# risingwavelabs/risingwave

Measured on NVIDIA H100. Metric: Nexmark q7/q8-shaped streaming HashJoin input rows/s, higher is better.
Workload: dtype int64

## Files before the change

risingwave_b200/csrc/join.cu:

```cuda
#include <algorithm>
#include <cstdio>
#include <cstdlib>
#include <memory>
#include <mutex>
#include <thread>

#include <cub/device/device_radix_sort.cuh>
#include <cub/device/device_scan.cuh>

#include "common.cuh"

namespace rw {

#define J_EMPTY 0x8000000000000000ull
#define J_NIL 0x7fffffffu
#define J_DEAD 0x80000000u
#define J_MAX_OUT (2 * RW_MAX_COLS)
#define J_HDR 16
#define W_EMPTY 0x7fffffffull
#define W_COUNT_ONE (1ull << 33)
#define W_IL_LIVE (1ull << 31)
#define W_IL_DEAD (2ull << 31)
#define W_IL_MASK (3ull << 31)
__device__ __host__ __forceinline__ uint32_t W_head(uint64_t W) { return (uint32_t)(W & 0x7fffffffull); }
// ... 24 lines not shown
  int out_type[J_MAX_OUT];
  int out_width[J_MAX_OUT];
  int n_map[2];
  int map_in[2][J_MAX_OUT];
  int map_out[2][J_MAX_OUT];
  int need_degree[2];
  int append_only_optimize;
  int cond_cmp, cond_lhs, cond_rhs;
  int single_key, KW, SW;
  int strict;
};

struct JoinSideDev {
  uint8_t* recs;
  uint8_t* buckets;
  uint64_t cap;
  int stride;
  int bstride;
};

struct JoinStatus {
  unsigned long long out_rows;
  unsigned long long n_store;
  unsigned long long n_del;
  unsigned long long null_mask;
  unsigned long long n_keys[2];
  unsigned int err;
  unsigned int pad;
  unsigned long long n_in;
  unsigned long long log_next[2];
  unsigned long long n_dead[2];
  unsigned long long n_defer;
};

struct JoinOutDev {
  uint8_t* ops;
  uint8_t* vis;
  void* col[J_MAX_OUT];
  uint8_t* valid[J_MAX_OUT];
  int64_t capacity;
  const uint8_t* heap[2];
};

__device__ __host__ __forceinline__ bool jt_is_outer_side(int T, int S) { return T == RW_JOIN_FULL_OUTER || (T == RW_JOIN_LEFT_OUTER && S == 0) || (T == RW_JOIN_RIGHT_OUTER && S == 1); }
__device__ __host__ __forceinline__ bool jt_outer_side_null(int T, int S) { return T == RW_JOIN_FULL_OUTER || (T == RW_JOIN_LEFT_OUTER && S == 1) || (T == RW_JOIN_RIGHT_OUTER && S == 0); }
__device__ __host__ __forceinline__ bool jt_forward_exactly_once(int T, int S) { return ((T == RW_JOIN_LEFT_SEMI || T == RW_JOIN_LEFT_ANTI) && S == 0) || ((T == RW_JOIN_RIGHT_SEMI || T == RW_JOIN_RIGHT_ANTI) && S == 1); }
__device__ __host__ __forceinline__ bool jt_only_forward_matched_side(int T, int S) { return ((T == RW_JOIN_LEFT_SEMI || T == RW_JOIN_LEFT_ANTI) && S == 1) || ((T == RW_JOIN_RIGHT_SEMI || T == RW_JOIN_RIGHT_ANTI) && S == 0); }
__device__ __host__ __forceinline__ bool jt_is_semi(int T) { return T == RW_JOIN_LEFT_SEMI || T == RW_JOIN_RIGHT_SEMI; }
__device__ __host__ __forceinline__ bool jt_is_anti(int T) { return T == RW_JOIN_LEFT_ANTI || T == RW_JOIN_RIGHT_ANTI; }
__device__ __host__ __forceinline__ bool jt_forward_if_not_matched(int T, int S) { return (jt_is_anti(T) && jt_forward_exactly_once(T, S)) || jt_is_outer_side(T, S); }

struct RecHdr {
  uint32_t link, nullmask, seq, degree;
};
__device__ __forceinline__ uint8_t* rec_ptr(const JoinSideDev& s, uint32_t row) { return s.recs + (uint64_t)row * s.stride; }
__device__ __forceinline__ RecHdr* rec_hdr(const JoinSideDev& s, uint32_t row) { return (RecHdr*)rec_ptr(s, row); }

__device__ __forceinline__ uint64_t rec_key_word(const uint8_t* rec, int off, int width, int type) {
  ColRef cr;
  cr.data = rec + off;
  cr.valid_bits = nullptr;
  cr.valid_bytes = nullptr;
  cr.type = type;
  cr.width = width;
  return load_key_word(cr, 0);
}
// ... 1203 lines not shown
      if (!sg.p) {
        cudaError_t e = sg.reserve((size_t)U_SEG_RECS * 48);
        if (e != cudaSuccess) { cudaGetLastError(); return fail(RW_ERR_OOM, std::string("join log segment: ") + cudaGetErrorString(e)); }
        stalls++;
      }
      void* ptr = sg.p;
      RW_CUDA(cudaMemcpyAsync(table.as<uint8_t>() + segs.size() * sizeof(void*), &ptr, sizeof(void*), cudaMemcpyHostToDevice, st));
      segs.push_back(std::move(sg));
    }
    return RW_OK;
  }
};

struct JoinSideHost {
  int n_cols = 0;
  std::vector<int> types;
  SegLog log;
  GrowBuf recs;
  DevBuf slots;
  DevBuf pools;
  int stride = 0, bstride = 0;
  uint64_t row_cap = 0;
  uint64_t n_rows = 0;
  uint64_t slot_cap = 0;
  uint64_t keys_upper = 0;
};

struct JoinPending {
  int S = 0, set = 0, grid = 0;
  DevChunk ch;
  cudaStream_t st = nullptr;
  int64_t out_base = 0;
  bool plain = true, counted = false, sync_done = false;
  bool alias_u = false;
  uint32_t pool_chunk = 0;
  uint64_t seq_base = 0, ids_before = 0, keys_before = 0;
  unsigned long long tag = 0;
  int64_t rows = 0;
  unsigned long long nullm = 0;
};

struct rwgpu_join {
  JoinPlanDev plan;
  DevBuf plan_dev, status;
  PinnedBuf status_host;
  JoinSideHost side[2];
  cudaStream_t stream = nullptr, s_h2d = nullptr, s_d2h = nullptr;
  cudaEvent_t ev_h2d[8] = {nullptr}, ev_main[8] = {nullptr};
  std::vector<int> out_types;
  int chunk_size = 1024;
  bool fast_inner = false;
  bool w8_ok[2] = {false, false};
  W8Plan w8[2];
  bool uni = false;
  int uni_is = 1;
  DevBuf uni_buckets, uni_counters;
  uint64_t uni_cap = 0, uni_keys = 0, uni_keys_exact = 0;
  uint64_t uni_dead[2] = {0, 0};
  uint64_t compactions = 0;
  DevBuf uni_wk_entry, uni_wk_mask;
  int64_t uni_wk_cap = 0;
  JoinPending pending[2];
  int n_pending = 0;
  cudaEvent_t pend_ev[2] = {nullptr, nullptr};
  cudaStream_t last_st = nullptr;
  cudaEvent_t order_ev = nullptr;
  bool wm_pending[2] = {false, false};
  int wm_key_pos[2] = {0, 0};
  int64_t wm_value[2] = {0, 0};
  uint64_t wm_cleanings = 0;
  uint64_t launches = 0;
  uint64_t seq = 0;
  unsigned long long status_tag = 0;
  unsigned long long call_null_mask = 0;
  bool out_rows_cumulative = false;
  KernelProf prof;
  DevBuf sk, sk_alt, packed, offs, mslot, gtable, cub_tmp;
  int64_t scratch_rows = 0;
  uint64_t gcap = 0;
  size_t cub_bytes = 0;
  struct OutSet {
    DevBuf out_ops, out_vis, out_col[J_MAX_OUT], out_valid[J_MAX_OUT], out_bits[J_MAX_OUT], out_visbits;
    int64_t out_cap = 0;
    unsigned long long valid_dirty = 0;
  } oset[2];
  int cur = 0;
  OutSet& os() { return oset[cur]; }
  struct HostPending {
    bool active = false;
    rwgpu_out* out = nullptr;
    std::vector<rw_column> in_cols;
    std::vector<int> alias_src;
    int64_t n = 0, host_cap = 0;
  } hpend[2];
// ... 154 lines not shown

static JoinOutDev out_dev(rwgpu_join* h) {
  JoinOutDev o;
  memset(&o, 0, sizeof(o));
  o.ops = h->os().out_ops.as<uint8_t>();
  o.vis = h->os().out_vis.as<uint8_t>();
  for (size_t k = 0; k < h->out_types.size(); k++) { o.col[k] = h->os().out_col[k].p; o.valid[k] = h->os().out_valid[k].as<uint8_t>(); }
  o.capacity = h->os().out_cap;
  o.heap[0] = h->var_heap[0].as<uint8_t>();
  o.heap[1] = h->var_heap[1].as<uint8_t>();
  return o;
}

__global__ void join_status_to_host_kernel(JoinStatus* src, JoinStatus* dst_host, unsigned long long tag, int reset) {
  join_status_publish(src, dst_host, tag, reset);
}
static int join_read_status(rwgpu_join* h, cudaStream_t st, JoinStatus* out, int reset = 1, unsigned long long tag = 0) {
  JoinStatus* host = h->status_host.as<JoinStatus>();
  if (tag) {
    RW_CUDA(cudaStreamSynchronize(st));
    if (*(volatile unsigned long long*)(host + 1) == tag) {
      memcpy(out, host, sizeof(JoinStatus));
      return RW_OK;
    }
  }
  join_status_to_host_kernel<<<1, 1, 0, st>>>(h->status.as<JoinStatus>(), host, 0ull, reset);
  RW_CUDA(cudaGetLastError());
  h->launches++;
  RW_CUDA(cudaStreamSynchronize(st));
  memcpy(out, host, sizeof(JoinStatus));
  return RW_OK;
}

static int join_check_err(rwgpu_join* h, const JoinStatus& s, cudaStream_t st) {
  if (!s.err) return RW_OK;
  unsigned int e = s.err;
  cudaMemsetAsync(&h->status.as<JoinStatus>()->err, 0, sizeof(unsigned int), st);
  if (e & JERR_DOUBLE_DELETE) return fail(RW_ERR_INCONSISTENT, "removing a join state entry but it is not in the cache");
  if (e & JERR_APPEND_ONLY_MULTI) return fail(RW_ERR_INCONSISTENT, "append-only optimisation: more than one matched row");
  if (e & JERR_STORE_CAPACITY) return fail(RW_ERR_CUDA, "internal: join record store capacity");
  if (e & JERR_BAD_COUNT) return fail(RW_ERR_INVALID, "device row count out of range");
  return fail(RW_ERR_CUDA, "internal: join output capacity");
}

static UniDev uni_dev(rwgpu_join* h) {
  UniDev t;
  t.buckets = h->uni_buckets.as<uint8_t>();
  t.cap = h->uni_cap;
  unsigned long long* ctr = h->uni_counters.as<unsigned long long>();
  for (int s = 0; s < 2; s++) {
    t.log[s] = h->side[s].log.table.as<uint8_t*>();
    t.log_cap[s] = h->side[s].log.cap();
    t.pools[s] = h->side[s].pools.as<uint2>();
    t.log_next[s] = ctr + s;
    t.n_dead[s] = ctr + 2 + s;
  }
  t.is = h->uni_is;
  return t;
}

static int uni_alloc_buckets(rwgpu_join* h, DevBuf& buf, uint64_t cap) {
  RW_CUDA(buf.reserve((cap + 2) * 64));
  uni_init_kernel<<<jgrid((int64_t)cap + 2, 256), 256, 0, h->stream>>>(buf.as<uint8_t>(), 0, cap + 2);
  RW_CUDA(cudaGetLastError());
  h->launches++;
  return RW_OK;
}

static int uni_grow_table(rwgpu_join* h, uint64_t need_keys) {
  if (need_keys * U_LOAD_INV <= h->uni_cap) return RW_OK;
  if (h->uni_keys_exact * U_LOAD_INV <= h->uni_cap && need_keys * 10 <= h->uni_cap * 9) return RW_OK;
  uint64_t ncap = h->uni_cap;
  while (ncap < need_keys * 2 * U_LOAD_INV) ncap <<= 1;
  RW_CUDA(cudaDeviceSynchronize());
  DevBuf nb;
  int rc = uni_alloc_buckets(h, nb, ncap);
  if (rc != RW_OK) return rc;
  uni_rehash_kernel<<<jgrid((int64_t)h->uni_cap + 2, 256), 256, 0, h->stream>>>(h->uni_buckets.as<uint8_t>(), h->uni_cap, nb.as<uint8_t>(), ncap);
  RW_CUDA(cudaGetLastError());
  h->launches++;
  RW_CUDA(cudaStreamSynchronize(h->stream));
  h->uni_buckets = std::move(nb);
  h->uni_cap = ncap;
  return RW_OK;
}

static int uni_compact(rwgpu_join* h, int s) {
  JoinSideHost& sd = h->side[s];
  RW_CUDA(cudaDeviceSynchronize());
  SegLog fresh;
  const uint64_t live_upper = sd.n_rows > h->uni_dead[s] ? sd.n_rows - h->uni_dead[s] : 0;
  int rc = fresh.ensure(std::max<uint64_t>(live_upper, 1), h->stream);
  if (rc != RW_OK) { set_error(""); return RW_OK; }
  unsigned long long* ctr = h->uni_counters.as<unsigned long long>();
  RW_CUDA(cudaMemsetAsync(ctr + 4, 0, 8, h->stream));
  uni_compact_kernel<<<jgrid((int64_t)h->uni_cap + 2, 256), 256, 0, h->stream>>>(uni_dev(h), s, fresh.table.as<uint8_t*>(), ctr + 4);
  RW_CUDA(cudaGetLastError());
  h->launches++;
  unsigned long long live = 0;
  RW_CUDA(cudaMemcpyAsync(&live, ctr + 4, 8, cudaMemcpyDeviceToHost, h->stream));
  RW_CUDA(cudaStreamSynchronize(h->stream));
  std::swap(sd.log.segs, fresh.segs);
  {
    DevBuf t2 = std::move(sd.log.table);
    sd.log.table = std::move(fresh.table);
    fresh.table = std::move(t2);
// ... 5 lines not shown
  RW_CUDA(cudaMemcpyAsync(ctr + s, &live, 8, cudaMemcpyHostToDevice, h->stream));
  RW_CUDA(cudaMemcpyAsync(ctr + 2 + s, &zero, 8, cudaMemcpyHostToDevice, h->stream));
  RW_CUDA(cudaMemsetAsync(sd.pools.p, 0, sd.pools.bytes, h->stream));
  RW_CUDA(cudaStreamSynchronize(h->stream));
  h->compactions++;
  return RW_OK;
}

static int join_order(rwgpu_join* h, cudaStream_t st) {
  if (h->last_st && h->last_st != st) {
    if (!h->order_ev) RW_CUDA(cudaEventCreateWithFlags(&h->order_ev, cudaEventDisableTiming));
    RW_CUDA(cudaEventRecord(h->order_ev, h->last_st));
    RW_CUDA(cudaStreamWaitEvent(st, h->order_ev, 0));
  }
  h->last_st = st;
  return RW_OK;
}

static int uni_tail_grid(int64_t n) {
  static int max_blocks = 0;
  if (!max_blocks) {
    int dev = 0, sms = 0, per_sm = 0;
    cudaGetDevice(&dev);
    cudaDeviceGetAttribute(&sms, cudaDevAttrMultiProcessorCount, dev);
    int a = 0, b = 0;
    cudaOccupancyMaxActiveBlocksPerMultiprocessor(&a, uni_tail_kernel<false>, 256, 0);
    cudaOccupancyMaxActiveBlocksPerMultiprocessor(&b, uni_tail_kernel<true>, 256, 0);
    per_sm = std::max(1, std::min(std::min(a, b), 3));
    max_blocks = std::max(1, sms * per_sm);
  }
  return (int)std::max<int64_t>(1, std::min<int64_t>((n + 255) / 256, max_blocks));
}

static int uni_launch_main(rwgpu_join* h, const JoinPending& pd, bool probe_only, unsigned long long tag) {
  UniDev t = uni_dev(h);
  const JoinPlanDev* pdev = h->plan_dev.as<JoinPlanDev>();
  JoinStatus* ds = h->status.as<JoinStatus>();
  int S = pd.S;
  const bool is_row = S == h->uni_is;
  JoinOutDev od = out_dev(h);
  UniWork wk;
  wk.entry = h->uni_wk_entry.as<UniDefer>();
  wk.mask = h->uni_wk_mask.as<uint8_t>();
  W8Plan w = h->w8[S];
  h->prof.begin(pd.st);
  if (pd.plain) {
    PlainChunk pc;
    pc.ops = pd.ch.ops;
    for (int c = 0; c < 4; c++) pc.c[c] = c < w.n_u ? (const unsigned long long*)pd.ch.cols[c].data : nullptr;
    pc.key = (const unsigned long long*)pd.ch.cols[w.key_col].data;
    pc.n = pd.ch.n;
    pc.n_dev = pd.ch.n_dev;
    UniOwn own;
    own.log = t.log[S];
    own.log_cap = t.log_cap[S];
    own.pools = t.pools[S];
    own.log_next = t.log_next[S];
    PlainOut po;
    po.ops = od.ops;
    po.vis = od.vis;
    const int mkey = pd.alias_u ? h->w8[1 - S].key_col : -1;
    for (int c = 0; c < 4; c++) {
      po.ucol[c] = (!pd.alias_u && c < w.n_u && w.u_out[c] >= 0) ? (unsigned long long*)od.col[w.u_out[c]] : nullptr;
      po.mcol[c] = (c != mkey && c < w.n_m && w.m_out[c] >= 0) ? (unsigned long long*)od.col[w.m_out[c]] : nullptr;
    }
    po.capacity = od.capacity;
    auto hot = probe_only ? (is_row ? uni_hot_kernel<true, true> : uni_hot_kernel<true, false>)
                          : (is_row ? uni_hot_kernel<false, true> : uni_hot_kernel<false, false>);
    hot<<<pd.grid, JF_BLOCK, 0, pd.st>>>(pc, t.buckets, t.cap, own, po, wk, ds, pd.seq_base, pd.out_base, pd.pool_chunk);
  } else {
    if (probe_only) uni_slow_kernel<true><<<jgrid(pd.ch.n, 256), 256, 0, pd.st>>>(pdev, w, S, pd.ch, t, od, ds, pd.seq_base, pd.out_base);
    else uni_slow_kernel<false><<<jgrid(pd.ch.n, 256), 256, 0, pd.st>>>(pdev, w, S, pd.ch, t, od, ds, pd.seq_base, pd.out_base);
  }
  h->prof.end(pd.st);
  RW_CUDA(cudaGetLastError());
  DevChunk chv = pd.ch;
  uint64_t seq_base = pd.seq_base;
  int64_t out_base = pd.out_base;
  JoinStatus* slot = (JoinStatus*)(h->status_host.as<uint8_t>() + 512 * pd.set);
  int reset = 3;
  unsigned int* done = (unsigned int*)(h->uni_counters.as<unsigned long long>() + 6);
  const int tg = uni_tail_grid(pd.ch.n);
  if (probe_only) uni_tail_kernel<true><<<tg, 256, 0, pd.st>>>(pdev, w, S, chv, t, od, wk, ds, seq_base, out_base, slot, tag, reset, done);
  else uni_tail_kernel<false><<<tg, 256, 0, pd.st>>>(pdev, w, S, chv, t, od, wk, ds, seq_base, out_base, slot, tag, reset, done);
  RW_CUDA(cudaGetLastError());
  h->launches += 2;
  return RW_OK;
}

static int join_plain_chunk(DevChunk* ch, bool device_count, cudaStream_t st, bool* plain) {
  *plain = ch->vis_bits == nullptr;
  for (int c = 0; c < ch->n_cols && *plain; c++)
    *plain = !ch->cols[c].valid_bits && !ch->cols[c].valid_bytes && (((uintptr_t)ch->cols[c].data & 7) == 0);
  if (!ch->n_dev || (device_count && *plain)) return RW_OK;
  int64_t nh = 0;
  RW_CUDA(cudaMemcpyAsync(&nh, ch->n_dev, sizeof(nh), cudaMemcpyDeviceToHost, st));
  RW_CUDA(cudaStreamSynchronize(st));
  if (nh < 0 || nh > ch->n) return fail(RW_ERR_INVALID, "device row count out of range");
  ch->n = nh;
  ch->n_dev = nullptr;
  return RW_OK;
}

static int uni_enqueue(rwgpu_join* h, int S, const DevChunk& ch_in, cudaStream_t st, int64_t out_base, bool alias_ok, JoinPending* pd) {
  DevChunk ch = ch_in;
  bool plain_cols;
  int rc = join_plain_chunk(&ch, true, st, &plain_cols);
  if (rc != RW_OK) return rc;
  const bool counted = ch.n_dev != nullptr;
  const int64_t n = ch.n;
  JoinSideHost& own = h->side[S];
  const int grid = (int)std::max<int64_t>(1, std::min<int64_t>((n + 63) / 64, U_MAX_GRID));
  uint32_t pool_chunk = 32;
  while (pool_chunk < 256 && (int64_t)pool_chunk * grid * 8 < 4 * n) pool_chunk <<= 1;
  const uint64_t id_slack = (uint64_t)grid * 8 * pool_chunk;
  rc = join_grow_store(h, S, own.n_rows + (uint64_t)n + id_slack);
  if (rc != RW_OK) return rc;
  rc = uni_grow_table(h, h->uni_keys + (uint64_t)n);
  if (rc != RW_OK) return rc;
  rc = join_ensure_out(h, out_base + n + std::max<int64_t>(n / 2, 4096), st, out_base);
  if (rc != RW_OK) return rc;
  if (plain_cols && n > h->uni_wk_cap) {
    RW_CUDA(cudaDeviceSynchronize());
    const int64_t cap = n + n / 4 + 64;
    RW_CUDA(h->uni_wk_entry.reserve((size_t)cap * sizeof(UniDefer)));
    RW_CUDA(h->uni_wk_mask.reserve((size_t)(cap + 7) / 8 + 16));
    h->uni_wk_cap = cap;
  }
  rc = join_order(h, st);
  if (rc != RW_OK) return rc;
  pd->S = S;
  pd->ch = ch;
  pd->st = st;
  pd->out_base = out_base;
  pd->set = h->cur;
  pd->plain = plain_cols;
  pd->counted = counted;
  pd->alias_u = alias_ok && plain_cols && !counted && out_base == 0 && h->var_in[S].empty();
  pd->grid = grid;
  pd->pool_chunk = pool_chunk;
  pd->seq_base = h->seq;
  pd->tag = ++h->status_tag;
  pd->ids_before = own.n_rows;
  pd->keys_before = h->uni_keys;
  h->seq += (uint64_t)n;
  own.n_rows += (uint64_t)n + id_slack;
  h->uni_keys += (uint64_t)n;
  rc = uni_launch_main(h, *pd, false, pd->tag);
  if (rc != RW_OK) return rc;
  if (!h->pend_ev[pd->set]) RW_CUDA(cudaEventCreateWithFlags(&h->pend_ev[pd->set], cudaEventDisableTiming));
  RW_CUDA(cudaEventRecord(h->pend_ev[pd->set], st));
  return RW_OK;
}

static int uni_finish(rwgpu_join* h, const JoinPending& pd, int64_t* out_rows, unsigned long long* null_mask, bool* aliased = nullptr) {
  cudaStream_t st = pd.st;
  JoinStatus* ds = h->status.as<JoinStatus>();
  JoinStatus* slot = (JoinStatus*)(h->status_host.as<uint8_t>() + 512 * pd.set);
  JoinStatus hs;
  RW_CUDA(cudaEventSynchronize(h->pend_ev[pd.set]));
  int rc;
  if (*(volatile unsigned long long*)(slot + 1) != pd.tag) return fail(RW_ERR_CUDA, "join status block was not published");
  memcpy(&hs, slot, sizeof(JoinStatus));
  unsigned int err = hs.err;
  const unsigned long long first_null = hs.null_mask;
  const bool first_match = hs.pad != 0;
  const unsigned long long first_del = hs.n_del;
  const bool redone = (hs.err & JERR_OUT_CAPACITY) != 0;
  if (redone) {
    const int64_t extras = (int64_t)hs.out_rows, n = pd.ch.n;
    RW_CUDA(cudaMemsetAsync(&ds->err, 0, 4, st));
    rc = join_ensure_out(h, pd.out_base + n + extras + (int64_t)pd.grid * 8 * U_XCHUNK, st, pd.out_base);
    if (rc != RW_OK) return rc;
    const unsigned long long tag2 = ++h->status_tag;
    rc = uni_launch_main(h, pd, true, tag2);
    if (rc != RW_OK) return rc;
    RW_CUDA(cudaStreamSynchronize(st));
    if (*(volatile unsigned long long*)(slot + 1) != tag2) return fail(RW_ERR_CUDA, "join status block was not published");
    memcpy(&hs, slot, sizeof(JoinStatus));
    err = (err & ~JERR_OUT_CAPACITY) | hs.err;
    hs.null_mask |= first_null & ~(1ull << 63);
    hs.pad = hs.pad || first_match;
    hs.n_del = first_del;
  }
  for (int s = 0; s < 2; s++) h->uni_dead[s] = hs.n_dead[s];
  {
    JoinSideHost& own = h->side[pd.S];
    const uint64_t n = (uint64_t)pd.ch.n, slack = (uint64_t)pd.grid * 8 * pd.pool_chunk;
    const uint64_t rows_now = hs.log_next[pd.S] + (own.n_rows - (pd.ids_before + n + slack));
    const uint64_t keys_now = hs.n_keys[0] + (h->uni_keys - (pd.keys_before + n));
    for (int i = 0; i < h->n_pending; i++) {
      h->pending[i].ids_before += rows_now - own.n_rows;
      h->pending[i].keys_before += keys_now - h->uni_keys;
    }
    own.n_rows = rows_now;
    h->uni_keys = keys_now;
    h->uni_keys_exact = hs.n_keys[0];
  }
  hs.err = err;
  rc = join_check_err(h, hs, st);
  if (rc != RW_OK) return rc;
  const int64_t n_eff = pd.counted ? (int64_t)hs.n_in : pd.ch.n;
  *out_rows = (hs.pad != 0 || hs.out_rows) ? n_eff + (int64_t)hs.out_rows : 0;
  h->call_null_mask |= hs.null_mask;
  *null_mask = h->call_null_mask;
  h->os().valid_dirty |= hs.null_mask & ((1ull << 63) - 1);
  if (hs.n_del) h->call_had_deletes = true;
  const bool alias = pd.alias_u && !redone && hs.out_rows == 0 && !h->call_had_deletes;
  if (pd.alias_u && !alias && *out_rows > 0) {
    const W8Plan& w = h->w8[pd.S];
    for (int c = 0; c < w.n_u; c++)
      if (w.u_out[c] >= 0)
        RW_CUDA(cudaMemcpyAsync(h->os().out_col[w.u_out[c]].p, pd.ch.cols[c].data, (size_t)pd.ch.n * 8, cudaMemcpyDeviceToDevice, st));
    const int mk = w.m_out[h->w8[1 - pd.S].key_col];
    if (mk >= 0)
      RW_CUDA(cudaMemcpyAsync(h->os().out_col[mk].p, pd.ch.cols[w.key_col].data, (size_t)pd.ch.n * 8, cudaMemcpyDeviceToDevice, st));
  }
  if (aliased) *aliased = alias;
  return RW_OK;
}

static int join_push_dev_uni(rwgpu_join* h, int S, const DevChunk& ch_in, cudaStream_t st, int64_t out_base, int64_t* out_rows,
                             unsigned long long* null_mask, bool* aliased) {
  if (h->n_pending) return fail(RW_ERR_INVALID, "collect the outstanding asynchronous pushes first");
  JoinPending pd;
  int rc = uni_enqueue(h, S, ch_in, st, out_base, aliased != nullptr, &pd);
  if (rc != RW_OK) return rc;
  return uni_finish(h, pd, out_rows, null_mask, aliased);
}

static int join_push_dev(rwgpu_join* h, int S, const DevChunk& ch_in, cudaStream_t st, int64_t out_base, int64_t* out_rows,
                         unsigned long long* null_mask, bool* aliased = nullptr) {
  *out_rows = 0;
// ... 317 lines not shown
  p.strict = d->strict_consistency;
  h->chunk_size = std::max(d->chunk_size > 0 ? d->chunk_size : 1024, 2);
  h->fast_inner = (T == RW_JOIN_INNER) && !p.append_only_optimize;
  for (int s2 = 0; s2 < 2 && h->fast_inner; s2++) {
    W8Plan& w = h->w8[s2];
    memset(&w, 0, sizeof(w));
    bool ok = p.single_key && p.cond_cmp == RW_CMP_NONE && p.n_cols[0] <= W8_MAXC && p.n_cols[1] <= W8_MAXC;
    for (int side = 0; side < 2 && ok; side++)
      for (int c = 0; c < p.n_cols[side]; c++) ok = ok && p.col_width[side][c] == 8 && p.col_off[side][c] == J_HDR + 8 * c;
    ok = ok && !type_is_float(p.col_type[s2][p.key_col[s2][0]]);
    w.n_u = p.n_cols[s2];
    w.n_m = p.n_cols[1 - s2];
    w.key_col = p.key_col[s2][0];
    for (int c = 0; c < W8_MAXC; c++) { w.u_out[c] = -1; w.m_out[c] = -1; }
    for (int i = 0; i < p.n_map[s2] && ok; i++) {
      if (w.u_out[p.map_in[s2][i]] >= 0) ok = false;
      w.u_out[p.map_in[s2][i]] = (int8_t)p.map_out[s2][i];
    }
    for (int i = 0; i < p.n_map[1 - s2] && ok; i++) {
      if (w.m_out[p.map_in[1 - s2][i]] >= 0) ok = false;
      w.m_out[p.map_in[1 - s2][i]] = (int8_t)p.map_out[1 - s2][i];
    }
    h->w8_ok[s2] = ok;
  }

  h->uni = h->fast_inner && h->w8_ok[0] && h->w8_ok[1] && p.n_cols[0] <= 4 && p.n_cols[1] <= 4;
  h->uni_is = pk_in_jk[1] ? 1 : (pk_in_jk[0] ? 0 : 1);

  RW_CUDA(cudaStreamCreateWithFlags(&h->stream, cudaStreamNonBlocking));
  RW_CUDA(h->var_ctr.reserve(32));
  RW_CUDA(cudaMemsetAsync(h->var_ctr.p, 0, 32, h->stream));
  RW_CUDA(h->plan_dev.reserve(sizeof(JoinPlanDev)));
  RW_CUDA(cudaMemcpyAsync(h->plan_dev.p, &p, sizeof(p), cudaMemcpyHostToDevice, h->stream));
  RW_CUDA(h->status.reserve(sizeof(JoinStatus)));
  RW_CUDA(cudaMemsetAsync(h->status.p, 0, sizeof(JoinStatus), h->stream));
  RW_CUDA(h->status_host.reserve(1024));
  if (h->uni) {
    const uint64_t hint = std::max(d->left.row_capacity_hint, d->right.row_capacity_hint);
    uint64_t cap = 1024;
    while (cap * 4 < hint * 5 * U_LOAD_INV) cap <<= 1;
    h->uni_cap = cap;
    rc = uni_alloc_buckets(h, h->uni_buckets, cap);
    if (rc != RW_OK) return rc;
    RW_CUDA(h->uni_counters.reserve(8 * sizeof(unsigned long long)));
    RW_CUDA(cudaMemsetAsync(h->uni_counters.p, 0, 8 * sizeof(unsigned long long), h->stream));
    for (int s = 0; s < 2; s++) {
      h->side[s].stride = 48;
      h->last_st = h->stream;
      uint64_t rows = s == h->uni_is ? std::max<uint64_t>(4096, sd[s]->row_capacity_hint / 4) : std::max<uint64_t>(4096, 2 * sd[s]->row_capacity_hint);
      if (sd[s]->stored_rows_hint && s != h->uni_is) rows = std::max<uint64_t>(4096, sd[s]->stored_rows_hint);
      rc = join_grow_store(h, s, std::min<uint64_t>(rows, 0x40000000ull));
      if (rc != RW_OK) return rc;
      RW_CUDA(h->side[s].pools.reserve((size_t)U_MAX_GRID * (JF_BLOCK / 32) * sizeof(uint2)));
      RW_CUDA(cudaMemsetAsync(h->side[s].pools.p, 0, h->side[s].pools.bytes, h->stream));
    }
  }
  for (int s = 0; s < 2 && !h->uni; s++) {
    uint64_t hint = sd[s]->row_capacity_hint;
    uint64_t cap = 1024;
    while (cap * 4 < hint * 10) cap <<= 1;
    h->side[s].slot_cap = cap;
    rc = join_alloc_slots(h, s, h->side[s].slots, cap);
    if (rc != RW_OK) return rc;
    rc = join_grow_store(h, s, std::max<uint64_t>(1024, std::min<uint64_t>(2 * hint, 0x40000000ull)));
    if (rc != RW_OK) return rc;
  }
  RW_CUDA(cudaStreamSynchronize(h->stream));
  *out = guard.release();
// ... 792 lines not shown
```

risingwave_b200/csrc/join_uni.cuh:

```cuda
#pragma once
#include <cooperative_groups.h>

namespace rw {

#define U_NIL 0x7fffffffu
#define U_XCHUNK 64
#define U_MAX_GRID (RW_SMS * 4)
#define U_LOAD_INV 4

#define U_SEG_SHIFT 22
#define U_SEG_RECS (1u << U_SEG_SHIFT)
#define U_MAX_SEGS 512
struct UniDev {
  uint8_t* buckets;
  uint64_t cap;
  uint8_t* const* log[2];
  uint64_t log_cap[2];
  uint2* pools[2];
  unsigned long long* log_next[2];
  unsigned long long* n_dead[2];
  int is;
};

struct UniRec {
// ... 247 lines not shown

__device__ __forceinline__ ulonglong2 ld128_cg(const void* ptr) { return __ldcg((const ulonglong2*)ptr); }

struct PlainChunk {
  const uint8_t* ops;
  const unsigned long long* c[4];
  const unsigned long long* key;
  int64_t n;
  const int64_t* n_dev;
};
struct UniOwn {
  uint8_t* const* log;
  uint64_t log_cap;
  uint2* pools;
  unsigned long long* log_next;
};
struct PlainOut {
  uint8_t* ops;
  uint8_t* vis;
  unsigned long long* ucol[4];
  unsigned long long* mcol[4];
  int64_t capacity;
};
struct UniDefer {
  int64_t b;
  int64_t xpos;
  uint32_t cnt;
  uint32_t pad;
};
struct UniWork {
  UniDefer* entry;
  uint8_t* mask;
};

template <bool PROBE_ONLY, bool IS_ROW>
__global__ void __launch_bounds__(JF_BLOCK, 4) uni_hot_kernel(PlainChunk ch, uint8_t* buckets, uint64_t cap, UniOwn own, PlainOut o, UniWork wk,
                                                               JoinStatus* st, uint64_t seq_base, int64_t out_base, uint32_t pool_chunk) {
  int64_t n_rows = ch.n;
  if (ch.n_dev) {
    const int64_t nd = *ch.n_dev;
    if (nd < 0 || nd > ch.n) {
      if (blockIdx.x == 0 && threadIdx.x == 0) atomicOr(&st->err, JERR_BAD_COUNT);
      n_rows = 0;
    } else {
      n_rows = nd;
      if (blockIdx.x == 0 && threadIdx.x == 0) st->n_in = (unsigned long long)nd;
    }
  }
  const int lane = lane_id(), q = lane & 3, qlead = lane & ~3;
  const int64_t warp_global = ((int64_t)blockIdx.x * blockDim.x + threadIdx.x) >> 5;
  uint32_t pool_next = 0, pool_end = 0;
  if (!PROBE_ONLY) {
    const uint2 pl = own.pools[warp_global];
    pool_next = pl.x;
    pool_end = pl.y;
  }
  int64_t xnext = 0, xend = 0;
  const int64_t xarea = out_base + n_rows;
  const uint64_t mask = cap - 1;
  unsigned int new_keys = 0, n_del = 0;
  enum : unsigned { SEEN_MATCH = 1u, SEEN_HOLE = 2u, SEEN_DEFER = 4u, SEEN_SENTINEL = 8u, SEEN_POOL = 16u };
  unsigned seen = 0u;
  const unsigned long long* pa = (q & 1) ? ch.c[2] : ch.c[0];
  const unsigned long long* pb = (q & 1) ? ch.c[3] : ch.c[1];
  const unsigned long long* pk = ch.key;
  __shared__ unsigned long long* s_po[8];
  if (threadIdx.x < 8) {
    const int c = threadIdx.x;
    s_po[c] = c == 0 ? o.ucol[0] : c == 1 ? o.ucol[2] : c == 2 ? o.mcol[0] : c == 3 ? o.mcol[2]
            : c == 4 ? o.ucol[1] : c == 5 ? o.ucol[3] : c == 6 ? o.mcol[1] : o.mcol[3];
// ... 215 lines not shown
          else *(ulonglong2*)(bp + 16 + 16 * (q - 1)) = make_ulonglong2(va, vb);
        } else {
          ulonglong2 v;
          if (q == 1) { v.x = (unsigned long long)link; v.y = seq; }
          else { v.x = va; v.y = vb; }
          *(ulonglong2*)(recp + 16 * (q - 1)) = v;
        }
      }
    }
  }
#undef UNI_FETCH
  for (int64_t f = xnext + lane; f < xend; f += 32) { o.ops[xarea + f] = RW_OP_INSERT; o.vis[xarea + f] = 0; }
  if (xend > xnext) seen |= SEEN_HOLE;
  if (!PROBE_ONLY && lane == 0 && (seen & SEEN_POOL)) own.pools[warp_global] = make_uint2(pool_next, pool_end);
  unsigned long long flags = ((seen & SEEN_HOLE) ? (1ull << 63) : 0ull);
  const bool warp_match = __any_sync(0xffffffffu, (seen & SEEN_MATCH) != 0u);
  const bool warp_defer = __any_sync(0xffffffffu, (seen & SEEN_DEFER) != 0u);
  const bool warp_sentinel = __any_sync(0xffffffffu, (seen & SEEN_SENTINEL) != 0u);
  for (int d = 16; d > 0; d >>= 1) {
    flags |= __shfl_xor_sync(0xffffffffu, flags, d);
    new_keys += __shfl_xor_sync(0xffffffffu, new_keys, d);
    n_del += __shfl_xor_sync(0xffffffffu, n_del, d);
  }
  if (lane == 0) {
    if (flags && (__ldcg(&st->null_mask) & flags) != flags) atomicOr(&st->null_mask, flags);
    if (warp_match && __ldcg(&st->pad) == 0u) st->pad = 1u;
    {
      const unsigned long long want = (warp_defer ? 1ull : 0ull) | (warp_sentinel ? 2ull : 0ull);
      if (want && (__ldcg(&st->n_defer) & want) != want) atomicOr(&st->n_defer, want);
    }
    if (!PROBE_ONLY && new_keys) atomicAdd(&st->n_keys[0], (unsigned long long)new_keys);
    if (!PROBE_ONLY && n_del) atomicAdd(&st->n_del, (unsigned long long)n_del);
  }
}

template <bool PROBE_ONLY>
__device__ __forceinline__ void uni_deferred_body(const JoinPlanDev* __restrict__ p, const W8Plan& w, int S, const DevChunk& ch, const UniDev& t,
                                                  const JoinOutDev& o, const UniWork& wk, JoinStatus* st, uint64_t seq_base, int64_t out_base) {
  const int64_t n_rows = chunk_rows(ch);
  unsigned new_keys = 0;
  bool any_match = false, any_hole = false;
  for (int64_t r = blockIdx.x * (int64_t)blockDim.x + threadIdx.x; r < n_rows; r += (int64_t)gridDim.x * blockDim.x) {
    if (!((wk.mask[r >> 3] >> (r & 7)) & 1u)) continue;
    const UniDefer e = wk.entry[r];
    const uint8_t op = ch.ops[r];
    const int64_t pos = out_base + r;
    if (e.cnt == 0u) {
      uni_row_generic<PROBE_ONLY>(p, w, S, ch, r, op, t, o, st, seq_base + (uint64_t)r, pos, out_base + n_rows, new_keys, any_match, any_hole);
    } else {
      any_match = true;
      o.vis[pos] = 1;
      const bool ins = (op == RW_OP_INSERT || op == RW_OP_UPDATE_INSERT);
      uni_emit_matches(t, w, S, ch, r, ins ? RW_OP_INSERT : RW_OP_DELETE, e.b, e.cnt, o, st, pos, e.xpos);
    }
  }
  if (any_hole) atomicOr(&st->null_mask, 1ull << 63);
  if (any_match) st->pad = 1u;
  if (!PROBE_ONLY && new_keys) atomicAdd(&st->n_keys[0], (unsigned long long)new_keys);
}

__device__ __forceinline__ bool uni_pk_equal(const JoinPlanDev* p, int S, const uint64_t* c, uint32_t nmask, const DevChunk& ch, int64_t r) {
  for (int i = 0; i < p->n_pk[S]; i++) {
    const int k = p->pk_col[S][i];
    const bool n1 = (nmask >> k) & 1u, n2 = col_is_null(ch.cols[k], r);
    if (n1 != n2) return false;
    if (n1) continue;
    const uint64_t x = c[k], y = ((const uint64_t*)ch.cols[k].data)[r];
    if (x != y) {
      if (p->col_type[S][k] != RW_T_FLOAT64) return false;
      const double fx = __longlong_as_double((long long)x), fy = __longlong_as_double((long long)y);
      if (fx != fy && (fx == fx || fy == fy)) return false;
    }
  }
  return true;
}

__device__ __forceinline__ void uni_delete_body(const JoinPlanDev* __restrict__ p, int S, const DevChunk& ch, const UniDev& t, JoinStatus* st,
                                                uint64_t seq_base, int sentinel_mode) {
  const int64_t n_rows = chunk_rows(ch);
  const uint64_t SEQ56 = (1ull << 56) - 1;
  unsigned int dead_log = 0;
  const int64_t r_first = sentinel_mode == 2 ? (int64_t)threadIdx.x : blockIdx.x * (int64_t)blockDim.x + threadIdx.x;
  const int64_t r_step = sentinel_mode == 2 ? (int64_t)blockDim.x : (int64_t)gridDim.x * blockDim.x;
  for (int64_t r = r_first; r < n_rows; r += r_step) {
    const uint8_t op = ch.ops[r];
    if (!row_visible(ch, r, op) || !(op == RW_OP_DELETE || op == RW_OP_UPDATE_DELETE)) continue;
    const ColRef& kc = ch.cols[p->key_col[S][0]];
    const bool knull = col_is_null(kc, r);
    if (knull && !p->null_safe[0]) continue;
    const uint64_t key = knull ? 0ull : ((const uint64_t*)kc.data)[r];
    if (sentinel_mode && ((!knull && key == J_EMPTY) != (sentinel_mode == 2))) continue;
    const int64_t b = uni_find(t, key, knull);
    bool found = false;
    while (b >= 0 && !found) {
      int best_kind = 0;
      uint32_t best_id = U_NIL;
      uint64_t best_seq = 0;
      auto consider = [&](int kind, uint32_t id, uint64_t seq, const uint64_t* c, uint32_t nmask) {
        const uint64_t d = (seq - seq_base) & SEQ56;
        if (d < (uint64_t)n_rows && d >= (uint64_t)r) return;
        if (!uni_pk_equal(p, S, c, nmask, ch, r)) return;
        const uint64_t rank = d < (uint64_t)n_rows ? (1ull << 60) + d : (seq & SEQ56);
        if (best_kind == 0 || rank > best_seq) { best_kind = kind; best_id = id; best_seq = rank; }
      };
      uint32_t m;
      if (S == t.is) {
        const unsigned long long WI = __ldcg(ub_WI(t, b));
        if (W_istate(WI) == 1u) {
          const unsigned long long ih = __ldcg(ub_IH(t, b));
          uint64_t c[4];
          const ulonglong2 c01 = __ldcg((const ulonglong2*)(ub(t, b) + 32)), c23 = __ldcg((const ulonglong2*)(ub(t, b) + 48));
          c[0] = c01.x; c[1] = c01.y; c[2] = c23.x; c[3] = c23.y;
          consider(1, 0u, ih >> 8, c, (uint32_t)(ih & 0xffull));
        }
        m = W_head(WI);
      } else {
        m = __ldcg(ub_chead(t, b));
      }
      while (m != U_NIL) {
        const UniRec* rec = urec(t, S, m);
        const ulonglong2 h0 = __ldcg((const ulonglong2*)rec);
        const uint32_t lk = (uint32_t)h0.x;
        if (!(lk & J_DEAD)) {
          uint64_t c[4];
          const ulonglong2 c01 = __ldcg((const ulonglong2*)rec + 1), c23 = __ldcg((const ulonglong2*)rec + 2);
          c[0] = c01.x; c[1] = c01.y; c[2] = c23.x; c[3] = c23.y;
          consider(2, m, h0.y, c, (uint32_t)(h0.x >> 32));
        }
        m = lk & 0x7fffffffu;
      }
      if (best_kind == 0) break;
      if (best_kind == 1) {
        unsigned long long* Wp = ub_WI(t, b);
// ... 161 lines not shown
```

Baseline: 5.915 billion.

## Skip tail kernel via last-block status publish in hot join kernel

Adds a lazy path for the non-row side: the hot kernel's last-finishing block publishes the status block to pinned host memory itself. The tail kernel is launched on the host later only when deferred rows or deletes are flagged (an owed-tail tag). Status blocks and work buffers are now kept per pending set so the two in-flight chunks do not share counters. This removes one kernel launch per chunk on the common append-only path. In exchange it adds a grid-wide atomic completion counter, a possible synchronous catch-up tail launch, and a changed self-visibility bound in the delete-matching check.

```diff
diff --git a/risingwave_b200/csrc/join.cu b/risingwave_b200/csrc/join.cu
--- a/risingwave_b200/csrc/join.cu
+++ b/risingwave_b200/csrc/join.cu
@@ -80,6 +80,7 @@
   unsigned long long n_dead[2];
   unsigned long long n_defer;
 };
+static_assert(sizeof(JoinStatus) <= 128, "status block");
 
 struct JoinOutDev {
   uint8_t* ops;
@@ -1349,6 +1350,7 @@
   cudaStream_t st = nullptr;
   int64_t out_base = 0;
   bool plain = true, counted = false, sync_done = false;
+  bool lazy = false;
   bool alias_u = false;
   uint32_t pool_chunk = 0;
   uint64_t seq_base = 0, ids_before = 0, keys_before = 0;
@@ -1375,8 +1377,9 @@
   uint64_t uni_cap = 0, uni_keys = 0, uni_keys_exact = 0;
   uint64_t uni_dead[2] = {0, 0};
   uint64_t compactions = 0;
-  DevBuf uni_wk_entry, uni_wk_mask;
-  int64_t uni_wk_cap = 0;
+  DevBuf uni_wk_entry[2], uni_wk_mask[2];
+  int64_t uni_wk_cap[2] = {0, 0};
+  uint64_t uni_set_keys[2] = {0, 0};
   JoinPending pending[2];
   int n_pending = 0;
   cudaEvent_t pend_ev[2] = {nullptr, nullptr};
@@ -1597,10 +1600,10 @@
   return RW_OK;
 }
 
-static int join_check_err(rwgpu_join* h, const JoinStatus& s, cudaStream_t st) {
+static int join_check_err(rwgpu_join* h, const JoinStatus& s, cudaStream_t st, JoinStatus* ds = nullptr) {
   if (!s.err) return RW_OK;
   unsigned int e = s.err;
-  cudaMemsetAsync(&h->status.as<JoinStatus>()->err, 0, sizeof(unsigned int), st);
+  cudaMemsetAsync(&(ds ? ds : h->status.as<JoinStatus>())->err, 0, sizeof(unsigned int), st);
   if (e & JERR_DOUBLE_DELETE) return fail(RW_ERR_INCONSISTENT, "removing a join state entry but it is not in the cache");
   if (e & JERR_APPEND_ONLY_MULTI) return fail(RW_ERR_INCONSISTENT, "append-only optimisation: more than one matched row");
   if (e & JERR_STORE_CAPACITY) return fail(RW_ERR_CUDA, "internal: join record store capacity");
@@ -1623,6 +1626,10 @@
   t.is = h->uni_is;
   return t;
 }
+static JoinStatus* uni_status(rwgpu_join* h, int set) { return (JoinStatus*)(h->status.as<uint8_t>() + 256 * set); }
+static unsigned int* uni_done(rwgpu_join* h, int set) { return (unsigned int*)(h->status.as<uint8_t>() + 256 * set + 128); }
+static JoinStatus* uni_slot(rwgpu_join* h, int set) { return (JoinStatus*)(h->status_host.as<uint8_t>() + 512 * set); }
+static int uni_run_owed_tail(rwgpu_join* h, JoinPending* pd);
 
 static int uni_alloc_buckets(rwgpu_join* h, DevBuf& buf, uint64_t cap) {
   RW_CUDA(buf.reserve((cap + 2) * 64));
@@ -1637,6 +1644,10 @@
   if (h->uni_keys_exact * U_LOAD_INV <= h->uni_cap && need_keys * 10 <= h->uni_cap * 9) return RW_OK;
   uint64_t ncap = h->uni_cap;
   while (ncap < need_keys * 2 * U_LOAD_INV) ncap <<= 1;
+  for (int i = 0; i < h->n_pending; i++) {
+    int rc = uni_run_owed_tail(h, &h->pending[i]);
+    if (rc != RW_OK) return rc;
+  }
   RW_CUDA(cudaDeviceSynchronize());
   DevBuf nb;
   int rc = uni_alloc_buckets(h, nb, ncap);
@@ -1708,16 +1719,16 @@
   return (int)std::max<int64_t>(1, std::min<int64_t>((n + 255) / 256, max_blocks));
 }
 
-static int uni_launch_main(rwgpu_join* h, const JoinPending& pd, bool probe_only, unsigned long long tag) {
+static int uni_launch_hot(rwgpu_join* h, const JoinPending& pd, bool probe_only, bool lazy, unsigned long long tag) {
   UniDev t = uni_dev(h);
   const JoinPlanDev* pdev = h->plan_dev.as<JoinPlanDev>();
-  JoinStatus* ds = h->status.as<JoinStatus>();
+  JoinStatus* ds = uni_status(h, pd.set);
   int S = pd.S;
   const bool is_row = S == h->uni_is;
   JoinOutDev od = out_dev(h);
   UniWork wk;
-  wk.entry = h->uni_wk_entry.as<UniDefer>();
-  wk.mask = h->uni_wk_mask.as<uint8_t>();
+  wk.entry = h->uni_wk_entry[pd.set].as<UniDefer>();
+  wk.mask = h->uni_wk_mask[pd.set].as<uint8_t>();
   W8Plan w = h->w8[S];
   h->prof.begin(pd.st);
   if (pd.plain) {
@@ -1741,26 +1752,63 @@
       po.mcol[c] = (c != mkey && c < w.n_m && w.m_out[c] >= 0) ? (unsigned long long*)od.col[w.m_out[c]] : nullptr;
     }
     po.capacity = od.capacity;
+    UniPublish pub;
+    pub.slot = lazy ? uni_slot(h, pd.set) : nullptr;
+    pub.ctr = h->uni_counters.as<unsigned long long>();
+    pub.done = uni_done(h, pd.set) + 1;
+    pub.tag = tag;
+    pub.reset = 3;
     auto hot = probe_only ? (is_row ? uni_hot_kernel<true, true> : uni_hot_kernel<true, false>)
                           : (is_row ? uni_hot_kernel<false, true> : uni_hot_kernel<false, false>);
-    hot<<<pd.grid, JF_BLOCK, 0, pd.st>>>(pc, t.buckets, t.cap, own, po, wk, ds, pd.seq_base, pd.out_base, pd.pool_chunk);
+    hot<<<pd.grid, JF_BLOCK, 0, pd.st>>>(pc, t.buckets, t.cap, own, po, wk, ds, pd.seq_base, pd.out_base, pd.pool_chunk, pub);
   } else {
     if (probe_only) uni_slow_kernel<true><<<jgrid(pd.ch.n, 256), 256, 0, pd.st>>>(pdev, w, S, pd.ch, t, od, ds, pd.seq_base, pd.out_base);
     else uni_slow_kernel<false><<<jgrid(pd.ch.n, 256), 256, 0, pd.st>>>(pdev, w, S, pd.ch, t, od, ds, pd.seq_base, pd.out_base);
   }
   h->prof.end(pd.st);
   RW_CUDA(cudaGetLastError());
+  h->launches++;
+  return RW_OK;
+}
+
+static int uni_launch_tail(rwgpu_join* h, const JoinPending& pd, bool probe_only, unsigned long long tag) {
+  UniDev t = uni_dev(h);
+  const JoinPlanDev* pdev = h->plan_dev.as<JoinPlanDev>();
+  JoinStatus* ds = uni_status(h, pd.set);
+  const int S = pd.S;
+  JoinOutDev od = out_dev(h);
+  UniWork wk;
+  wk.entry = h->uni_wk_entry[pd.set].as<UniDefer>();
+  wk.mask = h->uni_wk_mask[pd.set].as<uint8_t>();
+  W8Plan w = h->w8[S];
   DevChunk chv = pd.ch;
-  uint64_t seq_base = pd.seq_base;
-  int64_t out_base = pd.out_base;
-  JoinStatus* slot = (JoinStatus*)(h->status_host.as<uint8_t>() + 512 * pd.set);
-  int reset = 3;
-  unsigned int* done = (unsigned int*)(h->uni_counters.as<unsigned long long>() + 6);
+  JoinStatus* slot = uni_slot(h, pd.set);
+  unsigned int* done = uni_done(h, pd.set);
   const int tg = uni_tail_grid(pd.ch.n);
-  if (probe_only) uni_tail_kernel<true><<<tg, 256, 0, pd.st>>>(pdev, w, S, chv, t, od, wk, ds, seq_base, out_base, slot, tag, reset, done);
-  else uni_tail_kernel<false><<<tg, 256, 0, pd.st>>>(pdev, w, S, chv, t, od, wk, ds, seq_base, out_base, slot, tag, reset, done);
+  if (probe_only) uni_tail_kernel<true><<<tg, 256, 0, pd.st>>>(pdev, w, S, chv, t, od, wk, ds, pd.seq_base, pd.out_base, slot, tag, 3, done);
+  else uni_tail_kernel<false><<<tg, 256, 0, pd.st>>>(pdev, w, S, chv, t, od, wk, ds, pd.seq_base, pd.out_base, slot, tag, 3, done);
   RW_CUDA(cudaGetLastError());
-  h->launches += 2;
+  h->launches++;
+  return RW_OK;
+}
+
+static int uni_launch_main(rwgpu_join* h, const JoinPending& pd, bool probe_only, unsigned long long tag) {
+  int rc = uni_launch_hot(h, pd, probe_only, false, tag);
+  if (rc != RW_OK) return rc;
+  return uni_launch_tail(h, pd, probe_only, tag);
+}
+
+static int uni_run_owed_tail(rwgpu_join* h, JoinPending* pd) {
+  if (!pd->lazy) return RW_OK;
+  RW_CUDA(cudaEventSynchronize(h->pend_ev[pd->set]));
+  if (*(volatile unsigned long long*)(uni_slot(h, pd->set) + 1) != (pd->tag | UNI_TAIL_OWED)) return RW_OK;
+  const int cur = h->cur;
+  h->cur = pd->set;
+  pd->tag = ++h->status_tag;
+  const int rc = uni_launch_tail(h, *pd, false, pd->tag);
+  h->cur = cur;
+  if (rc != RW_OK) return rc;
+  RW_CUDA(cudaStreamSynchronize(pd->st));
   return RW_OK;
 }
 
@@ -1796,12 +1844,13 @@
   if (rc != RW_OK) return rc;
   rc = join_ensure_out(h, out_base + n + std::max<int64_t>(n / 2, 4096), st, out_base);
   if (rc != RW_OK) return rc;
-  if (plain_cols && n > h->uni_wk_cap) {
+  const int set = h->cur;
+  if (plain_cols && n > h->uni_wk_cap[set]) {
     RW_CUDA(cudaDeviceSynchronize());
     const int64_t cap = n + n / 4 + 64;
-    RW_CUDA(h->uni_wk_entry.reserve((size_t)cap * sizeof(UniDefer)));
-    RW_CUDA(h->uni_wk_mask.reserve((size_t)(cap + 7) / 8 + 16));
-    h->uni_wk_cap = cap;
+    RW_CUDA(h->uni_wk_entry[set].reserve((size_t)cap * sizeof(UniDefer)));
+    RW_CUDA(h->uni_wk_mask[set].reserve((size_t)(cap + 7) / 8 + 16));
+    h->uni_wk_cap[set] = cap;
   }
   rc = join_order(h, st);
   if (rc != RW_OK) return rc;
@@ -1809,10 +1858,11 @@
   pd->ch = ch;
   pd->st = st;
   pd->out_base = out_base;
-  pd->set = h->cur;
+  pd->set = set;
   pd->plain = plain_cols;
   pd->counted = counted;
   pd->alias_u = alias_ok && plain_cols && !counted && out_base == 0 && h->var_in[S].empty();
+  pd->lazy = alias_ok && plain_cols && !counted && h->var_in[S].empty() && S != h->uni_is;
   pd->grid = grid;
   pd->pool_chunk = pool_chunk;
   pd->seq_base = h->seq;
@@ -1822,20 +1872,22 @@
   h->seq += (uint64_t)n;
   own.n_rows += (uint64_t)n + id_slack;
   h->uni_keys += (uint64_t)n;
-  rc = uni_launch_main(h, *pd, false, pd->tag);
+  rc = pd->lazy ? uni_launch_hot(h, *pd, false, true, pd->tag) : uni_launch_main(h, *pd, false, pd->tag);
   if (rc != RW_OK) return rc;
   if (!h->pend_ev[pd->set]) RW_CUDA(cudaEventCreateWithFlags(&h->pend_ev[pd->set], cudaEventDisableTiming));
   RW_CUDA(cudaEventRecord(h->pend_ev[pd->set], st));
   return RW_OK;
 }
 
-static int uni_finish(rwgpu_join* h, const JoinPending& pd, int64_t* out_rows, unsigned long long* null_mask, bool* aliased = nullptr) {
+static int uni_finish(rwgpu_join* h, const JoinPending& pd_in, int64_t* out_rows, unsigned long long* null_mask, bool* aliased = nullptr) {
+  JoinPending pd = pd_in;
   cudaStream_t st = pd.st;
-  JoinStatus* ds = h->status.as<JoinStatus>();
-  JoinStatus* slot = (JoinStatus*)(h->status_host.as<uint8_t>() + 512 * pd.set);
+  JoinStatus* ds = uni_status(h, pd.set);
+  JoinStatus* slot = uni_slot(h, pd.set);
   JoinStatus hs;
   RW_CUDA(cudaEventSynchronize(h->pend_ev[pd.set]));
-  int rc;
+  int rc = uni_run_owed_tail(h, &pd);
+  if (rc != RW_OK) return rc;
   if (*(volatile unsigned long long*)(slot + 1) != pd.tag) return fail(RW_ERR_CUDA, "join status block was not published");
   memcpy(&hs, slot, sizeof(JoinStatus));
   unsigned int err = hs.err;
@@ -1864,17 +1916,19 @@
     JoinSideHost& own = h->side[pd.S];
     const uint64_t n = (uint64_t)pd.ch.n, slack = (uint64_t)pd.grid * 8 * pd.pool_chunk;
     const uint64_t rows_now = hs.log_next[pd.S] + (own.n_rows - (pd.ids_before + n + slack));
-    const uint64_t keys_now = hs.n_keys[0] + (h->uni_keys - (pd.keys_before + n));
+    h->uni_set_keys[pd.set] = hs.n_keys[0];
+    const uint64_t keys_exact = h->uni_set_keys[0] + h->uni_set_keys[1];
+    const uint64_t keys_now = keys_exact + (h->uni_keys - (pd.keys_before + n));
     for (int i = 0; i < h->n_pending; i++) {
       h->pending[i].ids_before += rows_now - own.n_rows;
       h->pending[i].keys_before += keys_now - h->uni_keys;
     }
     own.n_rows = rows_now;
     h->uni_keys = keys_now;
-    h->uni_keys_exact = hs.n_keys[0];
+    h->uni_keys_exact = keys_exact;
   }
   hs.err = err;
-  rc = join_check_err(h, hs, st);
+  rc = join_check_err(h, hs, st, ds);
   if (rc != RW_OK) return rc;
   const int64_t n_eff = pd.counted ? (int64_t)hs.n_in : pd.ch.n;
   *out_rows = (hs.pad != 0 || hs.out_rows) ? n_eff + (int64_t)hs.out_rows : 0;
@@ -2258,8 +2312,8 @@
   RW_CUDA(cudaMemsetAsync(h->var_ctr.p, 0, 32, h->stream));
   RW_CUDA(h->plan_dev.reserve(sizeof(JoinPlanDev)));
   RW_CUDA(cudaMemcpyAsync(h->plan_dev.p, &p, sizeof(p), cudaMemcpyHostToDevice, h->stream));
-  RW_CUDA(h->status.reserve(sizeof(JoinStatus)));
-  RW_CUDA(cudaMemsetAsync(h->status.p, 0, sizeof(JoinStatus), h->stream));
+  RW_CUDA(h->status.reserve(512));
+  RW_CUDA(cudaMemsetAsync(h->status.p, 0, 512, h->stream));
   RW_CUDA(h->status_host.reserve(1024));
   if (h->uni) {
     const uint64_t hint = std::max(d->left.row_capacity_hint, d->right.row_capacity_hint);
diff --git a/risingwave_b200/csrc/join_uni.cuh b/risingwave_b200/csrc/join_uni.cuh
--- a/risingwave_b200/csrc/join_uni.cuh
+++ b/risingwave_b200/csrc/join_uni.cuh
@@ -303,10 +303,19 @@
   UniDefer* entry;
   uint8_t* mask;
 };
+#define UNI_TAIL_OWED (1ull << 63)
+struct UniPublish {
+  JoinStatus* slot;
+  const unsigned long long* ctr;
+  unsigned int* done;
+  unsigned long long tag;
+  int reset;
+};
 
 template <bool PROBE_ONLY, bool IS_ROW>
 __global__ void __launch_bounds__(JF_BLOCK, 4) uni_hot_kernel(PlainChunk ch, uint8_t* buckets, uint64_t cap, UniOwn own, PlainOut o, UniWork wk,
-                                                               JoinStatus* st, uint64_t seq_base, int64_t out_base, uint32_t pool_chunk) {
+                                                               JoinStatus* st, uint64_t seq_base, int64_t out_base, uint32_t pool_chunk,
+                                                               UniPublish pub) {
   int64_t n_rows = ch.n;
   if (ch.n_dev) {
     const int64_t nd = *ch.n_dev;
@@ -588,6 +597,42 @@
     if (!PROBE_ONLY && new_keys) atomicAdd(&st->n_keys[0], (unsigned long long)new_keys);
     if (!PROBE_ONLY && n_del) atomicAdd(&st->n_del, (unsigned long long)n_del);
   }
+  if (pub.slot) {
+    __shared__ bool s_last;
+    __syncthreads();
+    if (threadIdx.x == 0) {
+      __threadfence();
+      s_last = atomicAdd(pub.done, 1u) == gridDim.x - 1;
+    }
+    __syncthreads();
+    if (s_last && threadIdx.x == 0) {
+      __threadfence();
+      pub.done[0] = 0u;
+      JoinStatus s;
+      s.out_rows = __ldcg(&st->out_rows);
+      s.n_store = __ldcg(&st->n_store);
+      s.n_del = __ldcg(&st->n_del);
+      s.null_mask = __ldcg(&st->null_mask);
+      s.n_keys[0] = __ldcg(&st->n_keys[0]);
+      s.n_keys[1] = __ldcg(&st->n_keys[1]);
+      s.err = __ldcg(&st->err);
+      s.pad = __ldcg(&st->pad);
+      s.n_in = __ldcg(&st->n_in);
+      s.log_next[0] = __ldcg(&pub.ctr[0]);
+      s.log_next[1] = __ldcg(&pub.ctr[1]);
+      s.n_dead[0] = __ldcg(&pub.ctr[2]);
+      s.n_dead[1] = __ldcg(&pub.ctr[3]);
+      s.n_defer = __ldcg(&st->n_defer);
+      if (s.n_defer != 0ull || s.n_del != 0ull) {
+        *(unsigned long long*)(pub.slot + 1) = pub.tag | UNI_TAIL_OWED;
+      } else {
+        *pub.slot = s;
+        *(unsigned long long*)(pub.slot + 1) = pub.tag;
+        if (pub.reset & 1) { st->n_store = 0ull; st->null_mask = 0ull; }
+        if (pub.reset & 2) { st->out_rows = 0ull; st->pad = 0u; st->n_in = 0ull; }
+      }
+    }
+  }
 }
 
 template <bool PROBE_ONLY>
@@ -654,7 +699,7 @@
       uint64_t best_seq = 0;
       auto consider = [&](int kind, uint32_t id, uint64_t seq, const uint64_t* c, uint32_t nmask) {
         const uint64_t d = (seq - seq_base) & SEQ56;
-        if (d < (uint64_t)n_rows && d >= (uint64_t)r) return;
+        if (d < (1ull << 55) && d >= (uint64_t)r) return;
         if (!uni_pk_equal(p, S, c, nmask, ch, r)) return;
         const uint64_t rank = d < (uint64_t)n_rows ? (1ull << 60) + d : (seq & SEQ56);
         if (best_kind == 0 || rank > best_seq) { best_kind = kind; best_id = id; best_seq = rank; }
```

New measurement: 6.289 billion, median of 6. +6.3%, better.
